# Youngju-Na/UFORecon

Hardware: AMD Instinct MI355X
Metric: rays/s (per-ray volume-rendering path, 64+64 hierarchical samples, DTU-shaped 3-view 512x640) (higher is better)
Workload: dtype f32; 1 GPU; configs[1]: full 512x640 frame = 327680 rays, 3 source views, 64+64 samples, rays sharded by row tiles over 1 GPU(s), depth/RGB tiles all-gathered; rays_per_frame=327680, chunk_rays=4096, side_streams=3

## Files before the change

### uforecon_amd/csrc/ray_transformer.hip

```cpp
#include "bwd_tape.h"
#include "ufr_internal.h"
#include "weight_stream_f16.h"

namespace ufr {

__device__ __forceinline__ void load_ray_tile(const float* __restrict__ token0, const int* __restrict__ tok_row,
                                              const float* __restrict__ order_pe, size_t tok_base, int s_base, int g,
                                              int j, f32x4 (&x)[6]) {
  const float* row = token0 + (tok_row ? (size_t)tok_row[tok_base + j] : tok_base + j) * UFR_TOKEN_DIM;
#pragma unroll
  for (int t = 0; t < 5; ++t) x[t] = ld4(row + 16 * t + 4 * g);
  const float* pe = order_pe + (size_t)(s_base + j) * 8 + 2 * g;
  x[5] = f32x4{pe[0], pe[1], 0.f, 0.f};
}

template <int VW, int VB, int C, class WS>
__device__ __forceinline__ void layer_norm88(f32x4 (&tt)[C][6], const WS& ws, int g, float eps, float asc, f32x4 (*XH)[6] = nullptr, float* RS = nullptr) {
#pragma unroll
  for (int c = 0; c < C; ++c) {
    f32x4 (&t)[6] = tt[c];
    float s = 0.f;
#pragma unroll
    for (int i = 0; i < 5; ++i) s += (t[i][0] + t[i][1]) + (t[i][2] + t[i][3]);
    s += t[5][0] + t[5][1];
    const float mean = sum_groups(s) * (1.f / 88.f);
    float q = 0.f;
#pragma unroll
    for (int i = 0; i < 6; ++i)
#pragma unroll
      for (int r = 0; r < 4; ++r) {
        if (i < 5 || r < 2) {
          float d = t[i][r] - mean;
          q = fmaf(d, d, q);
        }
      }
    const float rstd = fast_rsqrt(sum_groups(q) * (1.f / 88.f) + eps);
    if (RS) RS[c] = rstd * asc;
#pragma unroll
    for (int i = 0; i < 6; ++i) {
      const f32x4 gw = vec_frag<VW>(ws, i, g), gb = vec_frag<VB>(ws, i, g);
#pragma unroll
      for (int r = 0; r < 4; ++r) {
        const float xh = (t[i][r] - mean) * rstd;
        if (XH) XH[c][i][r] = (i == 5 && r >= 2) ? 0.f : xh;
        t[i][r] = xh * gw[r] + gb[r];
      }
    }
  }
}

constexpr int kRtBlock = 256;
constexpr int kRtMinW = 2;
constexpr int kRtWaves = kRtBlock / 64;

#ifdef UFR_PHASE_TIMING
__device__ unsigned long long g_rt_phase[32];
#define UFR_RT_PHASE(i)                                                                \
  {                                                                                    \
    const unsigned long long t_now = __builtin_readcyclecounter();                     \
    rt_acc[i] += t_now - rt_prev;                                                      \
    rt_prev = t_now;                                                                   \
  }
#else
#define UFR_RT_PHASE(i)
#endif

template <bool LOWP, bool TAPE = false>
__global__ void __launch_bounds__(kRtBlock, TAPE ? 2 : kRtMinW) ray_transformer_kernel(const float* __restrict__ packed,
                                                                  const float* __restrict__ token0,
                                                                  const int* __restrict__ tok_row,
                                                                  const float* __restrict__ order_pe, int RN, int SN,
                                                                  float* __restrict__ srdf,
                                                                  float* __restrict__ ray_out,
                                                                  int* __restrict__ status, float* __restrict__ tape = nullptr,
                                                                  float* __restrict__ ray_state = nullptr) {
  extern __shared__ __attribute__((aligned(16))) char smem[];
  auto ws = wstream_f16_begin<kRtWaves, LOWP>(packed, smem);
  wstream_f16_prime<B_RT1, kRtWaves>(ws);
  const int lane = threadIdx.x & 63, g = lane >> 4, j = lane & 15;
  const int ray_raw = (blockIdx.x * blockDim.x + threadIdx.x) >> 6;
  const bool valid = ray_raw < RN;
  const int ray = valid ? ray_raw : RN - 1;
  const int n_tiles = SN / 16;
  const int n_iter = n_tiles;
  const auto sc = scalar_file<false, ray_scalars_offset()>(ws);
  const float xs_x = sc[RS_XS_X];
  const float k_dsc = sc[RS_K_DSC], k_l2e = sc[RS_K_L2E], q_dsc = sc[RS_Q_DSC], q_l2e = sc[RS_Q_L2E];
  const float inv_len = uniform_f32(sc[RS_V_DSC] / (float)SN), f_len = uniform_f32((float)SN * sc[RS_V_ASC]);
  const bool pow2_len = (SN & (SN - 1)) == 0;

#ifdef UFR_PHASE_TIMING
  unsigned long long rt_acc[16] = {};
  unsigned long long rt_prev = __builtin_readcyclecounter();
#endif
  f32x4 KV[8], KVT[TAPE ? 8 : 1];
#pragma unroll
  for (int h = 0; h < 8; ++h) KV[h] = splat4(0.f);
#pragma unroll
  for (int h = 0; h < (TAPE ? 8 : 1); ++h) KVT[h] = splat4(0.f);
  for (int it = 0; it < n_iter; ++it) {
    constexpr int C = 1;
    const bool wrap = it + 1 < n_iter;
    const bool slot_ok = head11_slot(j) >= 0;
    f32x4 x[C][6], kt[C][8], vt[C][8];
    bool live[C];
#pragma unroll
    for (int c = 0; c < C; ++c) {
      const int tile = it * C + c;
      live[c] = tile < n_tiles;
      const int tl = live[c] ? tile : n_tiles - 1;
      load_ray_tile(token0, tok_row, order_pe, (size_t)ray * SN + tl * 16, tl * 16, g, j, x[c]);
#pragma unroll
      for (int h = 0; h < 8; ++h) { kt[c][h] = splat4(0.f); vt[c][h] = splat4(0.f); }
    }
    {
      BWords<C> cur;
      split_units<0, 0, 4 * C>(x, cur, xs_x);
      static_for<3>([&](auto si) __attribute__((always_inline)) {
        constexpr int s = decltype(si)::value;
        BStep b[C];
        bwords_to_bstep(cur, b);
        if constexpr (s < 2) {
          BWords<C> nxt;
          gemm_f16_panel<M_RT_K, s, C, kRtWaves, true>(ws, b, kt, wrap, [&](auto ti) __attribute__((always_inline)) {
            constexpr int to = decltype(ti)::value;
            split_units<s + 1, to * 4 * C / 8, (to + 1) * 4 * C / 8>(x, nxt, xs_x);
          });
          gemm_f16_panel<M_RT_V, s, C, kRtWaves, true>(ws, b, vt, wrap);
          cur = nxt;
        } else {
          gemm_f16_panel<M_RT_K, s, C, kRtWaves, true>(ws, b, kt, wrap);
          gemm_f16_panel<M_RT_V, s, C, kRtWaves, true>(ws, b, vt, wrap);
        }
      });
      probe_gemm(kt, ws);
      probe_gemm(vt, ws);
    }
    UFR_RT_PHASE(0)
    const float pad_v = (TAPE ? j == 3 : (j & 3) == 3) ? 1.f : 0.f;
#pragma unroll
    for (int c = 0; c < C; ++c) {
      float kk[8][4], vv[8][4];
      if (pow2_len) {
#pragma unroll
        for (int h = 0; h < 8; ++h)
#pragma unroll
          for (int r = 0; r < 4; ++r) vv[h][r] = vt[c][h][r] * inv_len;
      } else {
#pragma unroll
        for (int h = 0; h < 8; ++h)
#pragma unroll
          for (int r = 0; r < 4; ++r) vv[h][r] = vt[c][h][r] / f_len;
      }
      const bool k_ok = slot_ok && live[c];
#pragma unroll
      for (int h = 0; h < 8; ++h)
#pragma unroll
        for (int r = 0; r < 4; ++r) {
          const float e = elu1_acc(kt[c][h][r], k_dsc, k_l2e);
          kk[h][r] = k_ok ? e : 0.f;
          vv[h][r] = slot_ok ? vv[h][r] : pad_v;
        }
#pragma unroll
      for (int r = 0; r < 4; ++r) {
#pragma unroll
        for (int h = 0; h < 8; ++h) {
          KV[h] = mfma16(kk[h][r], vv[h][r], KV[h]);
          if constexpr (TAPE) KVT[h] = mfma16(vv[h][r], kk[h][r], KVT[h]);
        }
      }
    }
    wstream_f16_finish<B_RT1, kRtWaves>(ws, wrap);
    UFR_RT_PHASE(1)
  }

  if constexpr (TAPE) {
    if (valid) {
      float* st = ray_state + (size_t)ray * (kRayStateTiles * kTileFloats) + lane * 4;
#pragma unroll
      for (int h = 0; h < 8; ++h) { st4(st + h * kTileFloats, KV[h]); st4(st + (8 + h) * kTileFloats, KVT[h]); }
    }
  }
  wstream_f16_prime<B_RT2, kRtWaves>(ws);
  constexpr int C = 1;
  const int n_iter2 = TAPE ? n_iter + (n_iter & 1) : n_iter;
  typedef RayTapeLayout<LOWP> TapeL;
  for (int it = 0; it < n_iter2; ++it) {
    const bool wrap = it + 1 < n_iter2;
    char* const tape_blk = reinterpret_cast<char*>(tape) + ((size_t)ray * (n_iter2 / 2) + it / 2) * (TapeL::block_units * 512);
    auto tape_st = [&](int tile, f32x4 v) __attribute__((always_inline)) {
      if (valid) tile_store<TapeL>(tape_blk, tile, it & 1, lane, v);
    };
    f32x4 x[C][6], q[C][6], msg[C][6];
    bool live[C];
    int tbase[C];
#pragma unroll
    for (int c = 0; c < C; ++c) {
      const int tile = it * C + c;
      live[c] = tile < n_tiles;
      tbase[c] = (live[c] ? tile : n_tiles - 1) * 16;
      load_ray_tile(token0, tok_row, order_pe, (size_t)ray * SN + tbase[c], tbase[c], g, j, x[c]);
#pragma unroll
      for (int t = 0; t < 6; ++t) q[c][t] = splat4(0.f);
    }
    track_external(x, ws);
    gemm_f16<M_RT_Q, C, kRtWaves>(ws, x, q, wrap, xs_x);
    float zs_all[8];
    if constexpr (TAPE) {
#pragma unroll
      for (int t = 0; t < 6; ++t) {
        tape_st(RT_X + t, live[0] ? x[0][t] : splat4(0.f));
        f32x4 qq;
#pragma unroll
        for (int r = 0; r < 4; ++r) qq[r] = quad11(t, g, r) >= 0 ? elu1_acc(q[0][t][r], q_dsc, q_l2e) : 0.f;
        tape_st(RT_Q + t, qq);
      }
    }
    UFR_RT_PHASE(2)
#pragma unroll
    for (int c = 0; c < C; ++c) {
      static_for<8>([&](auto hi) __attribute__((always_inline)) {
        constexpr int h = decltype(hi)::value;
        f32x4 acc = splat4(0.f);
        static_for<3>([&](auto qi) __attribute__((always_inline)) {
          constexpr int qd = decltype(qi)::value, quad = 3 * h + qd;
          const float qq = (3 * g + qd < 11) ? elu1_acc(q[c][quad >> 2][quad & 3], q_dsc, q_l2e) : 0.f;
          acc = mfma16(KV[h][qd], qq, acc);
        });
        const float den = TAPE ? __shfl(acc[3], j) : acc[3];
        const float Z = fast_rcp(den + 1e-6f);
        const float zs = Z * (float)SN;
        if constexpr (TAPE) zs_all[h] = zs;
        static_for<3>([&](auto ri) __attribute__((always_inline)) {
          constexpr int rr = decltype(ri)::value, quad = 3 * h + rr;
          msg[c][quad >> 2][quad & 3] = acc[rr] * zs;
        });
      });
    }
    UFR_RT_PHASE(3)
    if constexpr (TAPE) {
#pragma unroll
      for (int t = 0; t < 6; ++t) tape_st(RT_MSG + t, msg[0][t]);
      tape_st(RT_ZS, f32x4{zs_all[0], zs_all[1], zs_all[2], zs_all[3]});
      tape_st(RT_ZS + 1, f32x4{zs_all[4], zs_all[5], zs_all[6], zs_all[7]});
    }
    f32x4 m[C][6];
#pragma unroll
    for (int c = 0; c < C; ++c)
#pragma unroll
      for (int t = 0; t < 6; ++t) m[c][t] = splat4(0.f);
    gemm_f16<M_RT_MERGE, C, kRtWaves>(ws, msg, m, wrap, sc[RS_M_XS]);
    UFR_RT_PHASE(4)
    float rstd1[C] = {}, rstd2[C] = {};
    if constexpr (TAPE) {
      f32x4 xh[C][6];
      layer_norm88<V_RT_N1W, V_RT_N1B, C>(m, ws, g, sc[RS_EPS1], sc[RS_M_ASC], xh, rstd1);
#pragma unroll
      for (int t = 0; t < 6; ++t) { tape_st(RT_XH1 + t, xh[0][t]); tape_st(RT_M + t, m[0][t]); }
    } else {
      layer_norm88<V_RT_N1W, V_RT_N1B, C>(m, ws, g, sc[RS_EPS1], 1.f);
    }
    UFR_RT_PHASE(5)

    f32x4 cat[C][12], hid[C][11], o[C][6];
#pragma unroll
    for (int c = 0; c < C; ++c) {
#pragma unroll
      for (int t = 0; t < 6; ++t) { cat[c][t] = x[c][t]; cat[c][6 + t] = m[c][t]; }
#pragma unroll
      for (int t = 0; t < 11; ++t) hid[c][t] = splat4(0.f);
    }
    gemm_f16<M_RT_MLP0, C, kRtWaves>(ws, cat, hid, wrap, xs_x);
    UFR_RT_PHASE(6)
#pragma unroll
    for (int c = 0; c < C; ++c) {
#pragma unroll
      for (int t = 0; t < 11; ++t)
#pragma unroll
        for (int r = 0; r < 4; ++r) hid[c][t][r] = relu_acc(hid[c][t][r]);
#pragma unroll
      for (int t = 0; t < 6; ++t) o[c][t] = splat4(0.f);
    }
    unsigned relu_bits[2] = {0u, 0u};
    if constexpr (TAPE) {
#pragma unroll
      for (int t = 0; t < 11; ++t) {
        tape_st(RT_HID + t, hid[0][t] * sc[RS_MLP0_DSC]);
#pragma unroll
        for (int r = 0; r < 4; ++r)
          if (hid[0][t][r] > 0.f) relu_bits[(4 * t + r) >> 5] |= 1u << ((4 * t + r) & 31);
      }
    }
    gemm_f16<M_RT_MLP2, C, kRtWaves>(ws, hid, o, wrap, sc[RS_M_MLP2]);
    UFR_RT_PHASE(7)
    if constexpr (TAPE) {
      f32x4 xh[C][6];
      layer_norm88<V_RT_N2W, V_RT_N2B, C>(o, ws, g, sc[RS_EPS2], sc[RS_MLP2_ASC], xh, rstd2);
#pragma unroll
      for (int t = 0; t < 6; ++t) tape_st(RT_XH2 + t, xh[0][t]);
    } else {
      layer_norm88<V_RT_N2W, V_RT_N2B, C>(o, ws, g, sc[RS_EPS2], 1.f);
    }
    UFR_RT_PHASE(8)
#pragma unroll
    for (int c = 0; c < C; ++c) {
#pragma unroll
      for (int t = 0; t < 6; ++t)
#pragma unroll
        for (int r = 0; r < 4; ++r) o[c][t][r] += x[c][t][r];
      if constexpr (TAPE) {
#pragma unroll
        for (int t = 0; t < 6; ++t) tape_st(RT_O + t, o[c][t]);
      }
      if (ray_out && valid && live[c]) {
        float* row = ray_out + ((size_t)ray * SN + tbase[c] + j) * UFR_RAY_DIM;
#pragma unroll
        for (int t = 0; t < 5; ++t) st4(row + 16 * t + 4 * g, o[c][t]);
        row[80 + 2 * g] = o[c][5][0];
        row[81 + 2 * g] = o[c][5][1];
      }
    }

    f32x4 d1[C][2], d2[C][1], d3[C][1];
#pragma unroll
    for (int c = 0; c < C; ++c) {
      d1[c][0] = vec_frag<V_DM_B0>(ws, 0, g) * sc[RS_DM0_ASC];
      d1[c][1] = vec_frag<V_DM_B0>(ws, 1, g) * sc[RS_DM0_ASC];
      d2[c][0] = vec_frag<V_DM_B2>(ws, 0, g) * sc[RS_DM2_ASC];
      d3[c][0] = vec_frag<V_DM_B4>(ws, 0, g) * sc[RS_DM4_ASC];
    }
    gemm_f16<M_DM0, C, kRtWaves>(ws, o, d1, wrap, sc[RS_DM0_XS]);
#pragma unroll
    for (int c = 0; c < C; ++c)
#pragma unroll
      for (int t = 0; t < 2; ++t)
#pragma unroll
        for (int r = 0; r < 4; ++r) d1[c][t][r] = relu_acc(d1[c][t][r]);
    gemm_f16<M_DM2, C, kRtWaves>(ws, d1, d2, wrap, sc[RS_M_DM2]);
#pragma unroll
    for (int c = 0; c < C; ++c)
#pragma unroll
      for (int r = 0; r < 4; ++r) d2[c][0][r] = relu_acc(d2[c][0][r]);
    if constexpr (TAPE) {
#pragma unroll
      for (int t = 0; t < 2; ++t) {
        tape_st(RT_D1 + t, d1[0][t] * sc[RS_DM0_DSC]);
#pragma unroll
        for (int r = 0; r < 4; ++r)
          if (d1[0][t][r] > 0.f) relu_bits[(44 + 4 * t + r) >> 5] |= 1u << ((44 + 4 * t + r) & 31);
      }
      tape_st(RT_D2, d2[0][0] * sc[RS_DM2_DSC]);
#pragma unroll
      for (int r = 0; r < 4; ++r)
        if (d2[0][0][r] > 0.f) relu_bits[1] |= 1u << (52 + r - 32);
      tape_st(RT_MISC, f32x4{rstd1[0], rstd2[0], __builtin_bit_cast(float, relu_bits[0]), __builtin_bit_cast(float, relu_bits[1])});
    }
    gemm_f16<M_DM4, C, kRtWaves>(ws, d2, d3, wrap, sc[RS_M_DM4]);
#pragma unroll
    for (int c = 0; c < C; ++c)
      if (g == 0 && valid && live[c]) srdf[(size_t)ray * SN + tbase[c] + j] = d3[c][0][0] * sc[RS_DM4_DSC];
    wstream_f16_finish<B_RT2, kRtWaves>(ws, wrap);
    UFR_RT_PHASE(9)
  }
  wstream_report_range(ws, status);
#ifdef UFR_PHASE_TIMING
  if (ray_raw == 5 && lane == 0)
    for (int i = 0; i < 16; ++i) g_rt_phase[i] += rt_acc[i];
#endif
}

template <bool LOWP, bool TAPE = false>
static hipError_t launch_rt(const float* packed, const float* token0, const int* tok_row, const float* order_pe, int RN,
                            int SN, float* srdf, float* ray_out, int* status, hipStream_t s, float* tape = nullptr,
                            float* ray_state = nullptr) {
  static LdsAttrOnce lds_attr;
  if (const hipError_t attr = lds_attr.set(reinterpret_cast<const void*>(&ray_transformer_kernel<LOWP, TAPE>), kF16LdsBytes); attr != hipSuccess) return attr;
  hipLaunchKernelGGL((ray_transformer_kernel<LOWP, TAPE>), dim3((RN + kRtWaves - 1) / kRtWaves), dim3(kRtBlock), kF16LdsBytes, s,
                     packed, token0, tok_row, order_pe, RN, SN, srdf, ray_out, status, tape, ray_state);
  return hipGetLastError();
}

hipError_t launch_ray_tape(const float* packed, const float* token0, const int* tok_row, const float* order_pe, int RN, int SN,
                           float* srdf, float* tape, float* ray_state, bool lowp, int* status, hipStream_t s) {
  if (SN % 16 != 0 || SN < 16) return hipErrorInvalidValue;
  return lowp ? launch_rt<true, true>(packed, token0, tok_row, order_pe, RN, SN, srdf, nullptr, status, s, tape, ray_state)
              : launch_rt<false, true>(packed, token0, tok_row, order_pe, RN, SN, srdf, nullptr, status, s, tape, ray_state);
}

hipError_t launch_ray_transformer(const float* packed, const float* token0, const int* tok_row, const float* order_pe,
                                  int RN, int SN, float* srdf, float* ray_out, bool lowp, int* status, hipStream_t s) {
  if (SN % 16 != 0 || SN < 16) return hipErrorInvalidValue;
  return lowp ? launch_rt<true>(packed, token0, tok_row, order_pe, RN, SN, srdf, ray_out, status, s)
              : launch_rt<false>(packed, token0, tok_row, order_pe, RN, SN, srdf, ray_out, status, s);
}

}

#ifdef UFR_PHASE_TIMING
extern "C" int ufr_debug_rt_phases(unsigned long long* out, int n, int reset) {
  unsigned long long h[32] = {};
  if (hipMemcpyFromSymbol(h, HIP_SYMBOL(ufr::g_rt_phase), sizeof(h)) != hipSuccess) return -1;
  for (int i = 0; i < n && i < 32; ++i) out[i] = h[i];
  if (reset) {
    unsigned long long z[32] = {};
    if (hipMemcpyToSymbol(HIP_SYMBOL(ufr::g_rt_phase), z, sizeof(z)) != hipSuccess) return -1;
  }
  return 0;
}
#endif
```

### uforecon_amd/csrc/ufr_layout_f16.h

```cpp
#pragma once
#include "ufr_layout.h"

namespace ufr {

constexpr int kPlanes = 2;
constexpr int kScaleExpWMin = -40, kScaleExpWMax = 24, kScaleExpXMin = -40, kScaleExpXMax = 12;
constexpr float kDefaultInputAbsMax = 4094.f;
constexpr int kF16ChunkFrags = 12;
constexpr int kF16Slots = 3;
constexpr int kF16Depth = 2;
static_assert(kF16Depth >= 1 && kF16Depth * kPlanes <= kF16ChunkFrags, "read-ahead must stay inside one chunk");

enum F16Stream { B_VT = 0, B_RT1 = 1, B_RT2 = 2, B_COUNT = 3, B_VTB = 3, B_RTB1 = 4, B_RTB2 = 5, B_ALL = 6 };
__host__ __device__ constexpr bool f16_mat_is_bf16(int m) { return m >= M_COUNT; }

struct Panel { int mat, s; };

__host__ __device__ constexpr int ksteps(int m) { return (mat_desc(m).n_in + 1) / 2; }

__host__ __device__ constexpr int f16_n_panels(int S) {
  return S == B_VT ? 3 * 3 + 3 + 5 + 5 + 3 + 1 + 1 : S == B_RT1 ? 6 : S == B_RT2 ? 3 + 3 + 6 + 6 + 3 + 1 + 1
       : S == B_VTB ? 1 + 1 + 3 + 5 + 3 + 3 * 3
       : S == B_RTB1 ? 1 + 1 + 3 + 6 + 3 + 3
       : 6 + 4 + 4;
}
__host__ __device__ constexpr Panel f16_panel(int S, int i) {
  if (S == B_VT) {
    if (i < 6) return {i % 2 == 0 ? M_VT_Q : M_VT_K, i / 2};
    if (i < 9) return {M_VT_V, i - 6};
    i -= 9;
    if (i < 3) return {M_VT_MERGE, i};
    i -= 3;
    if (i < 5) return {M_VT_MLP0, i};
    i -= 5;
    if (i < 5) return {M_VT_MLP2, i};
    i -= 5;
    if (i < 3) return {M_RW0, i};
    i -= 3;
    return {i == 0 ? M_RW2 : M_RW4, 0};
  }
  if (S == B_RT1) return {i % 2 == 0 ? M_RT_K : M_RT_V, i / 2};
  if (S == B_VTB) {
    if (i < 1) return {M_RW2T, 0};
    i -= 1;
    if (i < 1) return {M_RW0T, 0};
    i -= 1;
    if (i < 3) return {M_VT_MLP2T, i};
    i -= 3;
    if (i < 5) return {M_VT_MLP0T, i};
    i -= 5;
    if (i < 3) return {M_VT_MERGET, i};
    i -= 3;
    return {i < 3 ? M_VT_QT : i < 6 ? M_VT_KT : M_VT_VT, i % 3};
  }
  if (S == B_RTB1) {
    if (i < 1) return {M_DM2T, 0};
    i -= 1;
    if (i < 1) return {M_DM0T, 0};
    i -= 1;
    if (i < 3) return {M_RT_MLP2T, i};
    i -= 3;
    if (i < 6) return {M_RT_MLP0T, i};
    i -= 6;
    if (i < 3) return {M_RT_MERGET, i};
    i -= 3;
    return {M_RT_QT, i};
  }
  if (S == B_RTB2) {
    if (i < 6) return {i % 2 == 0 ? M_RT_K : M_RT_V, i / 2};
    i -= 6;
    return {i < 4 ? M_RT_KT : M_RT_VT, i % 4};
  }
  if (i < 3) return {M_RT_Q, i};
  i -= 3;
  if (i < 3) return {M_RT_MERGE, i};
  i -= 3;
  if (i < 6) return {M_RT_MLP0, i};
  i -= 6;
  if (i < 6) return {M_RT_MLP2, i};
  i -= 6;
  if (i < 3) return {M_DM0, i};
  i -= 3;
  return {i == 0 ? M_DM2 : M_DM4, 0};
}
__host__ __device__ constexpr int f16_mat_stream(int m) {
  return m >= M_DM2T ? ((m == M_RT_KT || m == M_RT_VT) ? B_RTB2 : B_RTB1)
         : m >= M_COUNT ? B_VTB
         : (m == M_RT_K || m == M_RT_V) ? B_RT1
         : (m == M_RT_Q || m == M_RT_MERGE || m == M_RT_MLP0 || m == M_RT_MLP2 || m == M_DM0 || m == M_DM2 || m == M_DM4)
             ? B_RT2
             : B_VT;
}
__host__ __device__ constexpr int f16_panel_frags(int S, int i) { return mat_desc(f16_panel(S, i).mat).n_out * kPlanes; }
__host__ __device__ constexpr int f16_panel_start(int S, int i) {
  int o = 0;
  for (int j = 0; j < i; ++j) o += f16_panel_frags(S, j);
  return o;
}
__host__ __device__ constexpr int f16_panel_index(int m, int s, int S = -1) {
  if (S < 0) S = f16_mat_stream(m);
  for (int i = 0; i < f16_n_panels(S); ++i)
    if (f16_panel(S, i).mat == m && f16_panel(S, i).s == s) return i;
  return -1;
}
__host__ __device__ constexpr int f16_stream_frags(int S) { return f16_panel_start(S, f16_n_panels(S)); }
__host__ __device__ constexpr int f16_stream_real_chunks(int S) { return (f16_stream_frags(S) + kF16ChunkFrags - 1) / kF16ChunkFrags; }
__host__ __device__ constexpr int f16_stream_chunks(int S) { return (f16_stream_real_chunks(S) + kF16Slots - 1) / kF16Slots * kF16Slots; }
__host__ __device__ constexpr int f16_stream_base_frags(int S) {
  int o = 0;
  for (int j = 0; j < S; ++j) o += f16_stream_chunks(j) * kF16ChunkFrags;
  return o;
}
constexpr int kF16FragsPadded = f16_stream_base_frags(B_COUNT);
constexpr int kF16Halfwords = kF16FragsPadded * 512;
constexpr int kF16Bytes = kF16FragsPadded * 1024;
constexpr int kBwdFragsPadded = f16_stream_base_frags(B_ALL) - kF16FragsPadded;
constexpr int kBwdHalfwords = kBwdFragsPadded * 512;
constexpr int kBwdBytes = kBwdFragsPadded * 1024;

__host__ __device__ constexpr int f16_col(int m, int s, int g, int i) {
  const MatDesc d = mat_desc(m);
  const int tile = 2 * s + (i >> 2);
  return tile < d.n_in ? col_map(d.cm, tile, g, i & 3, d.in_dim) : -1;
}

__host__ __device__ inline void plan_entry_f16(int h, int* param, int* elem, int* plane, int* is_bf16 = nullptr, int* mat = nullptr) {
  *param = -1; *elem = 0; *plane = 0;
  int f = h >> 9;
  const int lane = (h >> 3) & 63, i = h & 7;
  int S = 0;
  while (S + 1 < B_ALL && f >= f16_stream_base_frags(S + 1)) ++S;
  if (is_bf16) *is_bf16 = 0;
  if (mat) *mat = -1;
  f -= f16_stream_base_frags(S);
  if (f >= f16_stream_frags(S)) return;
  int pi = 0;
  while (f >= f16_panel_frags(S, pi)) { f -= f16_panel_frags(S, pi); ++pi; }
  const Panel p = f16_panel(S, pi);
  if (is_bf16) *is_bf16 = f16_mat_is_bf16(p.mat) ? 1 : 0;
  if (mat) *mat = p.mat;
  const MatDesc d = mat_desc(p.mat);
  const int to = f / kPlanes;
  *plane = f % kPlanes;
  const int row = row_map(d.rm, to, lane & 15, d.out_dim);
  const int col = f16_col(p.mat, p.s, lane >> 4, i);
  if (row >= 0 && col >= 0) { *param = d.param; *elem = d.trans ? col * d.k_raw + row : row * d.k_raw + col; }
}

}
```

### uforecon_amd/csrc/weight_stream_f16.h

```cpp
#pragma once
#include <type_traits>

#include "ufr_layout_f16.h"
#include "weight_stream.h"

namespace ufr {

typedef _Float16 f16x8 __attribute__((ext_vector_type(8)));
typedef _Float16 f16x2 __attribute__((ext_vector_type(2)));
typedef float f32x2 __attribute__((ext_vector_type(2)));
typedef unsigned u32x4 __attribute__((ext_vector_type(4)));
typedef int i32x4 __attribute__((ext_vector_type(4)));

constexpr int kF16RingBytes = kF16Slots * kF16ChunkFrags * 1024;
constexpr int kF16LdsBytes = kF16RingBytes + kVecBytes;

__device__ __forceinline__ void split_pair(float a, float b, float m, unsigned& h, unsigned& l) {
  if (__builtin_constant_p(a) && __builtin_constant_p(b) && a == 0.f && b == 0.f) {
    h = l = 0u;
    return;
  }
  asm("v_fma_mixlo_f16 %0, %1, %2, 0" : "=v"(h) : "v"(a), "s"(m));
  asm("v_fma_mixhi_f16 %0, %1, %2, 0" : "+v"(h) : "v"(b), "s"(m));
  asm("v_fma_mixlo_f16 %0, %1, %2, -%3 op_sel_hi:[0,0,1]" : "=v"(l) : "v"(a), "s"(m), "v"(h));
  asm("v_fma_mixhi_f16 %0, %1, %2, -%3 op_sel:[0,0,1] op_sel_hi:[0,0,1]" : "+v"(l) : "v"(b), "s"(m), "v"(h));
}

struct BStep { f16x8 p[kPlanes]; };

typedef __bf16 bf16x2 __attribute__((ext_vector_type(2)));
typedef __bf16 bf16x8 __attribute__((ext_vector_type(8)));
__device__ __forceinline__ void split_pair_bf16(float a, float b, unsigned& h, unsigned& l) {
  h = __builtin_bit_cast(unsigned, __builtin_convertvector(f32x2{a, b}, bf16x2));
  const float ah = __builtin_bit_cast(float, h << 16), bh = __builtin_bit_cast(float, h & 0xffff0000u);
  l = __builtin_bit_cast(unsigned, __builtin_convertvector(f32x2{a - ah, b - bh}, bf16x2));
}

template <bool LOWP, bool BF16 = false>
struct WStreamF16T {
  static constexpr bool lowp = LOWP;
  static constexpr bool bf16 = BF16;
  const char* src;
  char* ring;
  unsigned ring_lds;
  i32x4 rsrc;
  unsigned lds_wave;
  const f32x4* vecs;
  int wave, lane;
  unsigned long long bad_in, bad_out;
  f16x8 pre[kF16Depth][kPlanes];
};

typedef WStreamF16T<false> WStreamF16;
template <int NWAVES, bool LOWP = false, bool BF16 = false>
__device__ __forceinline__ WStreamF16T<LOWP, BF16> wstream_f16_begin(const float* __restrict__ packed, char* smem) {
  WStreamF16T<LOWP, BF16> ws;
  ws.lane = threadIdx.x & 63;
  ws.wave = __builtin_amdgcn_readfirstlane(threadIdx.x >> 6);
  ws.bad_in = ws.bad_out = 0ull;
  constexpr size_t kPlaneRegion = (size_t)blob_floats() * 4;
  ws.src = reinterpret_cast<const char*>(packed) + kPlaneRegion;
  ws.ring = smem;
  ws.ring_lds = __builtin_amdgcn_readfirstlane((unsigned)(size_t)(lds_ptr_t)smem);
  {
    const unsigned long long base = reinterpret_cast<unsigned long long>(ws.src) + (unsigned long long)ws.wave * 1024ull;
    ws.rsrc[0] = __builtin_amdgcn_readfirstlane((int)(unsigned)(base & 0xffffffffull));
    ws.rsrc[1] = __builtin_amdgcn_readfirstlane((int)(unsigned)((base >> 32) & 0xffffull));
    ws.rsrc[2] = -1;
    ws.rsrc[3] = 0x00020000;
    ws.lds_wave = ws.ring_lds + (unsigned)ws.wave * 1024u;
  }
  f32x4* v = reinterpret_cast<f32x4*>(smem + kF16RingBytes);
  ws.vecs = v;
  constexpr int voff = vec_region_offset(), n4 = vec_region_floats() / 4;
  const f32x4* vs = reinterpret_cast<const f32x4*>(packed + voff);
  for (int i = threadIdx.x; i < n4; i += NWAVES * 64) v[i] = vs[i];
  __syncthreads();
  return ws;
}

template <unsigned GOFF, unsigned LOFF>
__device__ __forceinline__ void lds_dma_piece(const i32x4& rsrc, unsigned lds_wave, unsigned lane_off) {
  unsigned soff;
  asm volatile("s_add_u32 m0, %3, %5\n\ts_mov_b32 %0, %4\n\tbuffer_load_dwordx4 %1, %2, %0 offen lds"
               : "=&s"(soff)
               : "v"(lane_off), "s"(rsrc), "s"(lds_wave), "n"(GOFF), "n"(LOFF)
               : "memory", "scc");
}

template <int S, int NWAVES, int CHK, int P0 = 0, int P1 = kF16ChunkFrags / NWAVES, class WS>
__device__ __forceinline__ void wstream_f16_fetch(const WS& ws) {
  static_assert(kF16ChunkFrags % NWAVES == 0, "chunk must split evenly over the fetching waves");
  if constexpr (P1 > P0) {
    constexpr size_t goff = ((size_t)f16_stream_base_frags(S) + (size_t)CHK * kF16ChunkFrags) * 1024;
    constexpr int soff = (CHK % kF16Slots) * (kF16ChunkFrags * 1024);
    const unsigned lane_off = ws.lane * 16;
    static_assert(goff + (size_t)kF16ChunkFrags * 1024 < (1ull << 31), "buffer offsets are 32-bit");
    static_for<P1 - P0>([&](auto ki) __attribute__((always_inline)) {
      constexpr unsigned k = P0 + decltype(ki)::value;
      lds_dma_piece<(unsigned)goff + k * NWAVES * 1024u, (unsigned)soff + k * NWAVES * 1024u>(ws.rsrc, ws.lds_wave, lane_off);
    });
  }
}

template <int S, int NWAVES, int CHK, class WS>
__device__ __forceinline__ void wstream_f16_barrier(const WS& ws, bool wrap) {
  constexpr int per_chunk = kF16ChunkFrags / NWAVES, ahead = kF16Slots - 1, n_chunks = f16_stream_chunks(S);
  constexpr int younger = (kF16Slots - 2) * per_chunk;
  if constexpr (younger == 0) {
    asm volatile("s_waitcnt vmcnt(0) lgkmcnt(0)" ::: "memory");
  } else if constexpr (CHK + ahead <= n_chunks) {
    asm volatile("s_waitcnt vmcnt(%0) lgkmcnt(0)" ::"n"(younger) : "memory");
  } else {
    if (wrap) asm volatile("s_waitcnt vmcnt(%0) lgkmcnt(0)" ::"n"(younger) : "memory");
    else asm volatile("s_waitcnt vmcnt(0) lgkmcnt(0)" ::: "memory");
  }
  __syncthreads();
}

template <int S, int NWAVES, int CHK, int P0 = 0, int P1 = kF16ChunkFrags / NWAVES, class WS>
__device__ __forceinline__ void wstream_f16_refill(const WS& ws, bool wrap) {
  constexpr int ahead = kF16Slots - 1, n_chunks = f16_stream_chunks(S);
  if constexpr (CHK + ahead < n_chunks) {
    wstream_f16_fetch<S, NWAVES, CHK + ahead, P0, P1>(ws);
  } else {
    if (wrap) wstream_f16_fetch<S, NWAVES, (CHK + ahead) % n_chunks, P0, P1>(ws);
  }
}

template <int S, int NWAVES, int CHK, class WS>
__device__ __forceinline__ void wstream_f16_open(const WS& ws, bool wrap) {
  wstream_f16_barrier<S, NWAVES, CHK>(ws, wrap);
  wstream_f16_refill<S, NWAVES, CHK>(ws, wrap);
}

template <int S, int NWAVES, class WS>
__device__ __forceinline__ void wstream_f16_finish(const WS& ws, bool wrap) {
  constexpr int real = f16_stream_real_chunks(S), pad = f16_stream_chunks(S) - real;
  static_for<pad>([&](auto ci) __attribute__((always_inline)) { wstream_f16_open<S, NWAVES, real + decltype(ci)::value>(ws, wrap); });
}

template <int S, int NWAVES, class WS>
__device__ __forceinline__ void wstream_f16_prime(const WS& ws) {
  static_for<kF16Slots - 1>([&](auto ci) __attribute__((always_inline)) { wstream_f16_fetch<S, NWAVES, decltype(ci)::value>(ws); });
}

template <int C, int N, class WS>
__device__ __forceinline__ void probe_gemm(const f32x4 (&out)[C][N], WS& ws) {
  bool bad = false;
#pragma unroll
  for (int c = 0; c < C; ++c) bad |= __builtin_amdgcn_class(out[c][0][0], 0x207);
  ws.bad_in |= __builtin_amdgcn_ballot_w64(bad);
}
template <int C, int N, class WS>
__device__ __forceinline__ void track_external(const f32x4 (&t)[C][N], WS& ws) {
  bool nan = false;
#pragma unroll
  for (int c = 0; c < C; ++c)
#pragma unroll
    for (int i = 0; i < N; ++i)
      nan |= __builtin_isunordered(t[c][i][0], t[c][i][1]) | __builtin_isunordered(t[c][i][2], t[c][i][3]);
  ws.bad_out |= __builtin_amdgcn_ballot_w64(nan);
}

template <class WS>
__device__ __forceinline__ void wstream_report_range(const WS& ws, int* __restrict__ status) {
  const int bits = (ws.bad_in ? 1 : 0) | (ws.bad_out ? 2 : 0);
  if (bits && ws.lane == 0) atomicOr(status, bits);
}

template <int V, class WS>
__device__ __forceinline__ f32x4 vec_frag(const WS& ws, int t, int g) {
  constexpr int base = (vec_offset(V) - vec_region_offset()) / 4;
  return ws.vecs[base + t * 4 + g];
}

__device__ __forceinline__ float uniform_f32(float v) {
  return __builtin_bit_cast(float, __builtin_amdgcn_readfirstlane(__builtin_bit_cast(int, v)));
}
template <bool LOCAL>
struct ScalarFile {
  float sv;
  __device__ __forceinline__ float operator[](int k) const {
    float v = sv;
    if constexpr (LOCAL) asm volatile("" : "+v"(v));
    return __builtin_bit_cast(float, __builtin_amdgcn_readlane(__builtin_bit_cast(int, v), k));
  }
};
template <bool LOCAL, int OFFSET, class WS>
__device__ __forceinline__ ScalarFile<LOCAL> scalar_file(const WS& ws) {
  constexpr int base = OFFSET - vec_region_offset();
  return ScalarFile<LOCAL>{reinterpret_cast<const float*>(ws.vecs)[base + (ws.lane & (kKernelScalars - 1))]};
}

__device__ __forceinline__ f32x4 mfma_f16(const f16x8& a, const f16x8& b, const f32x4& c) {
  return __builtin_amdgcn_mfma_f32_16x16x32_f16(a, b, c, 0, 0, 0);
}
template <bool BF>
__device__ __forceinline__ f32x4 mfma_planes(const f16x8& a, const f16x8& b, const f32x4& c) {
  if constexpr (BF)
    return __builtin_amdgcn_mfma_f32_16x16x32_bf16(__builtin_bit_cast(bf16x8, a), __builtin_bit_cast(bf16x8, b), c, 0, 0, 0);
  else
    return __builtin_amdgcn_mfma_f32_16x16x32_f16(a, b, c, 0, 0, 0);
}

constexpr int kHookValu = 6;
constexpr int kProducts = 3;
constexpr int kSetprio = 1;
struct NoHook {
  template <class T> __device__ __forceinline__ void operator()(T) const {}
};
template <int M, int S, int C, int NWAVES, bool SWAP = false, int STREAM = -1, class Hook = NoHook, class WS = WStreamF16>
__device__ __forceinline__ void gemm_f16_panel(WS& ws, const BStep (&b)[C], f32x4 (&out)[C][mat_desc(M).n_out],
                                              bool wrap, Hook&& hook = NoHook{}) {
  constexpr bool LOWP = WS::lowp;
  constexpr bool BF = f16_mat_is_bf16(M);
  constexpr int n_planes = LOWP ? 1 : kPlanes, n_products = LOWP ? 1 : kProducts;
  constexpr int n_out = mat_desc(M).n_out, ST = STREAM >= 0 ? STREAM : f16_mat_stream(M);
  static_assert(f16_panel_index(M, S, ST) >= 0, "not a panel of the stream");
  constexpr int F0 = f16_panel_start(ST, f16_panel_index(M, S, ST));
  const f16x8* lds = reinterpret_cast<const f16x8*>(ws.ring) + ws.lane;
  __builtin_amdgcn_s_setprio(kSetprio);
  static_for<n_out>([&](auto ti) __attribute__((always_inline)) {
    constexpr int to = decltype(ti)::value;
    constexpr int f = F0 + to * kPlanes;
    constexpr int sidx = f / kPlanes, n_stages = f16_stream_frags(ST) / kPlanes;
    __builtin_amdgcn_sched_barrier(0);
    auto read_stage = [&](auto si) __attribute__((always_inline)) {
      constexpr int s2 = decltype(si)::value, f2 = s2 * kPlanes;
      constexpr int chk = f2 / kF16ChunkFrags, in_chk = f2 % kF16ChunkFrags;
      constexpr int base = ((chk % kF16Slots) * kF16ChunkFrags + in_chk) * 64;
      constexpr int in_frags = f16_stream_frags(ST) - chk * kF16ChunkFrags;
      constexpr int n_st = (in_frags < kF16ChunkFrags ? in_frags : kF16ChunkFrags) / kPlanes, j = in_chk / kPlanes;
      constexpr int pieces = kF16ChunkFrags / NWAVES;
      if constexpr (in_chk == 0) wstream_f16_barrier<ST, NWAVES, chk>(ws, wrap);
      wstream_f16_refill<ST, NWAVES, chk, j * pieces / n_st, (j + 1) * pieces / n_st>(ws, wrap);
#pragma unroll
      for (int p = 0; p < n_planes; ++p) ws.pre[s2 % kF16Depth][p] = lds[base + p * 64];
    };
    if constexpr (sidx == 0)
      static_for<kF16Depth>([&](auto di) __attribute__((always_inline)) { read_stage(di); });
    f16x8 a[kPlanes];
#pragma unroll
    for (int p = 0; p < n_planes; ++p) a[p] = ws.pre[sidx % kF16Depth][p];
    if constexpr (sidx + kF16Depth < n_stages) read_stage(std::integral_constant<int, sidx + kF16Depth>{});
    __builtin_amdgcn_sched_barrier(0);
    hook(ti);
#pragma unroll
    for (int c = 0; c < C; ++c)
      static_for<n_products>([&](auto pi) __attribute__((always_inline)) {
        constexpr int pw[kProducts] = {1, 0, 0}, px[kProducts] = {0, 1, 0};
        constexpr int w = LOWP ? 0 : pw[decltype(pi)::value], x = LOWP ? 0 : px[decltype(pi)::value];
        out[c][to] = SWAP ? mfma_planes<BF>(b[c].p[x], a[w], out[c][to]) : mfma_planes<BF>(a[w], b[c].p[x], out[c][to]);
      });
    if constexpr (!std::is_same<std::decay_t<Hook>, NoHook>::value) {
#pragma unroll
      for (int i = 0; i < n_products * C; ++i) {
        __builtin_amdgcn_sched_group_barrier(0x008, 1, 0);
        __builtin_amdgcn_sched_group_barrier(0x002, kHookValu, 0);
      }
    }
#pragma unroll
    for (int c = 0; c < C; ++c) asm volatile("" : "+v"(out[c][to]));
  });
  __builtin_amdgcn_sched_barrier(0);
  __builtin_amdgcn_s_setprio(0);
}

template <int C>
struct BWords { unsigned w[C][kPlanes][4]; };

template <int S, int U0, int U1, bool BF = false, int C, int NIN>
__device__ __forceinline__ void split_units(const f32x4 (&in)[C][NIN], BWords<C>& bw, float m) {
  static_for<U1 - U0>([&](auto ui) __attribute__((always_inline)) {
    constexpr int u = U0 + decltype(ui)::value;
    constexpr int c = u / 4, half = (u >> 1) & 1, q = u & 1, tile = 2 * S + half;
    if constexpr (tile < NIN) {
      if constexpr (BF) split_pair_bf16(in[c][tile][2 * q], in[c][tile][2 * q + 1], bw.w[c][0][2 * half + q], bw.w[c][1][2 * half + q]);
      else split_pair(in[c][tile][2 * q], in[c][tile][2 * q + 1], m, bw.w[c][0][2 * half + q], bw.w[c][1][2 * half + q]);
    } else {
      bw.w[c][0][2 * half + q] = bw.w[c][1][2 * half + q] = 0u;
    }
  });
}

template <int C>
__device__ __forceinline__ void bwords_to_bstep(const BWords<C>& bw, BStep (&b)[C]) {
#pragma unroll
  for (int c = 0; c < C; ++c)
#pragma unroll
    for (int p = 0; p < kPlanes; ++p)
      b[c].p[p] = __builtin_bit_cast(f16x8, u32x4{bw.w[c][p][0], bw.w[c][p][1], bw.w[c][p][2], bw.w[c][p][3]});
}

__device__ __forceinline__ float elu1_acc(float a, float dsc, float dsc_l2e) {
  return a > 0.f ? __builtin_fmaf(a, dsc, 1.f) : __builtin_amdgcn_exp2f(dsc_l2e * a);
}
constexpr float kLog2e = 0x1.715476p+0f;

template <int M, int C, int NWAVES, int STREAM = -1, int NIN, class WS, class UHook = NoHook>
__device__ __forceinline__ void gemm_f16(WS& ws, const f32x4 (&in)[C][NIN], f32x4 (&out)[C][mat_desc(M).n_out],
                                        bool wrap, float m = 1.f, UHook&& uhook = NoHook{}) {
  static_assert(NIN == mat_desc(M).n_in, "input tile count");
  constexpr int n_out = mat_desc(M).n_out, NU = 4 * C;
  constexpr bool BF = f16_mat_is_bf16(M);
  constexpr bool kUser = !std::is_same<std::decay_t<UHook>, NoHook>::value;
  BWords<C> cur;
  split_units<0, 0, NU, BF>(in, cur, m);
  static_for<ksteps(M)>([&](auto si) __attribute__((always_inline)) {
    constexpr int s = decltype(si)::value;
    BStep b[C];
    bwords_to_bstep(cur, b);
    if constexpr (s + 1 < ksteps(M) && n_out >= 2) {
      BWords<C> nxt;
      gemm_f16_panel<M, s, C, NWAVES, false, STREAM>(ws, b, out, wrap, [&](auto ti) __attribute__((always_inline)) {
        constexpr int to = decltype(ti)::value;
        split_units<s + 1, to * NU / n_out, (to + 1) * NU / n_out, BF>(in, nxt, m);
        if constexpr (kUser) uhook(std::integral_constant<int, s * n_out + to>{});
      });
      cur = nxt;
    } else if constexpr (kUser) {
      gemm_f16_panel<M, s, C, NWAVES, false, STREAM>(ws, b, out, wrap, [&](auto ti) __attribute__((always_inline)) {
        uhook(std::integral_constant<int, s * n_out + decltype(ti)::value>{});
      });
      if constexpr (s + 1 < ksteps(M)) split_units<s + 1, 0, NU, BF>(in, cur, m);
    } else {
      gemm_f16_panel<M, s, C, NWAVES, false, STREAM>(ws, b, out, wrap);
      if constexpr (s + 1 < ksteps(M)) split_units<s + 1, 0, NU, BF>(in, cur, m);
    }
  });
  if constexpr (!BF) probe_gemm(out, ws);
}

}
```

Before: 2.604 million rays/s.

## Process two ray tiles per weight pass in RT1 with head-grouped virtual weight order

In the non-tape ray transformer first stage, each weight-stream pass now handles two 16-sample tiles (C=2) instead of one, and loops over head groups of two. The B_RT1 weight stream is fetched in a permuted virtual order so each head group's K/V panels arrive contiguously. This is meant to halve weight-streaming traffic and barrier count per tile while keeping accumulator register pressure bounded. The stream barriers also now skip padding pieces and compute exact vmcnt waits. The risks are added register pressure from C=2 and added complexity in the fetch and wait accounting.

```diff
diff --git a/uforecon_amd/csrc/ray_transformer.hip b/uforecon_amd/csrc/ray_transformer.hip
--- a/uforecon_amd/csrc/ray_transformer.hip
+++ b/uforecon_amd/csrc/ray_transformer.hip
@@ -75,7 +75,7 @@
                                                                   int* __restrict__ status, float* __restrict__ tape = nullptr,
                                                                   float* __restrict__ ray_state = nullptr) {
   extern __shared__ __attribute__((aligned(16))) char smem[];
-  auto ws = wstream_f16_begin<kRtWaves, LOWP>(packed, smem);
+  auto ws = wstream_f16_begin<kRtWaves, LOWP, false, !TAPE>(packed, smem);
   wstream_f16_prime<B_RT1, kRtWaves>(ws);
   const int lane = threadIdx.x & 63, g = lane >> 4, j = lane & 15;
   const int ray_raw = (blockIdx.x * blockDim.x + threadIdx.x) >> 6;
@@ -98,80 +98,150 @@
   for (int h = 0; h < 8; ++h) KV[h] = splat4(0.f);
 #pragma unroll
   for (int h = 0; h < (TAPE ? 8 : 1); ++h) KVT[h] = splat4(0.f);
-  for (int it = 0; it < n_iter; ++it) {
-    constexpr int C = 1;
-    const bool wrap = it + 1 < n_iter;
+  if constexpr (TAPE) {
+    for (int it = 0; it < n_iter; ++it) {
+      constexpr int C = 1;
+      const bool wrap = it + 1 < n_iter;
+      const bool slot_ok = head11_slot(j) >= 0;
+      f32x4 x[C][6], kt[C][8], vt[C][8];
+      bool live[C];
+#pragma unroll
+      for (int c = 0; c < C; ++c) {
+        const int tile = it * C + c;
+        live[c] = tile < n_tiles;
+        const int tl = live[c] ? tile : n_tiles - 1;
+        load_ray_tile(token0, tok_row, order_pe, (size_t)ray * SN + tl * 16, tl * 16, g, j, x[c]);
+#pragma unroll
+        for (int h = 0; h < 8; ++h) { kt[c][h] = splat4(0.f); vt[c][h] = splat4(0.f); }
+      }
+      {
+        BWords<C> cur;
+        split_units<0, 0, 4 * C>(x, cur, xs_x);
+        static_for<3>([&](auto si) __attribute__((always_inline)) {
+          constexpr int s = decltype(si)::value;
+          BStep b[C];
+          bwords_to_bstep(cur, b);
+          if constexpr (s < 2) {
+            BWords<C> nxt;
+            gemm_f16_panel<M_RT_K, s, C, kRtWaves, true>(ws, b, kt, wrap, [&](auto ti) __attribute__((always_inline)) {
+              constexpr int to = decltype(ti)::value;
+              split_units<s + 1, to * 4 * C / 8, (to + 1) * 4 * C / 8>(x, nxt, xs_x);
+            });
+            gemm_f16_panel<M_RT_V, s, C, kRtWaves, true>(ws, b, vt, wrap);
+            cur = nxt;
+          } else {
+            gemm_f16_panel<M_RT_K, s, C, kRtWaves, true>(ws, b, kt, wrap);
+            gemm_f16_panel<M_RT_V, s, C, kRtWaves, true>(ws, b, vt, wrap);
+          }
+        });
+        probe_gemm(kt, ws);
+        probe_gemm(vt, ws);
+      }
+      UFR_RT_PHASE(0)
+      const float pad_v = (TAPE ? j == 3 : (j & 3) == 3) ? 1.f : 0.f;
+#pragma unroll
+      for (int c = 0; c < C; ++c) {
+        float kk[8][4], vv[8][4];
+        if (pow2_len) {
+#pragma unroll
+          for (int h = 0; h < 8; ++h)
+#pragma unroll
+            for (int r = 0; r < 4; ++r) vv[h][r] = vt[c][h][r] * inv_len;
+        } else {
+#pragma unroll
+          for (int h = 0; h < 8; ++h)
+#pragma unroll
+            for (int r = 0; r < 4; ++r) vv[h][r] = vt[c][h][r] / f_len;
+        }
+        const bool k_ok = slot_ok && live[c];
+#pragma unroll
+        for (int h = 0; h < 8; ++h)
+#pragma unroll
+          for (int r = 0; r < 4; ++r) {
+            const float e = elu1_acc(kt[c][h][r], k_dsc, k_l2e);
+            kk[h][r] = k_ok ? e : 0.f;
+            vv[h][r] = slot_ok ? vv[h][r] : pad_v;
+          }
+#pragma unroll
+        for (int r = 0; r < 4; ++r) {
+#pragma unroll
+          for (int h = 0; h < 8; ++h) {
+            KV[h] = mfma16(kk[h][r], vv[h][r], KV[h]);
+            if constexpr (TAPE) KVT[h] = mfma16(vv[h][r], kk[h][r], KVT[h]);
+          }
+        }
+      }
+      wstream_f16_finish<B_RT1, kRtWaves>(ws, wrap);
+      UFR_RT_PHASE(1)
+    }
+  } else {
     const bool slot_ok = head11_slot(j) >= 0;
-    f32x4 x[C][6], kt[C][8], vt[C][8];
-    bool live[C];
-#pragma unroll
-    for (int c = 0; c < C; ++c) {
-      const int tile = it * C + c;
-      live[c] = tile < n_tiles;
-      const int tl = live[c] ? tile : n_tiles - 1;
-      load_ray_tile(token0, tok_row, order_pe, (size_t)ray * SN + tl * 16, tl * 16, g, j, x[c]);
-#pragma unroll
-      for (int h = 0; h < 8; ++h) { kt[c][h] = splat4(0.f); vt[c][h] = splat4(0.f); }
-    }
-    {
-      BWords<C> cur;
-      split_units<0, 0, 4 * C>(x, cur, xs_x);
-      static_for<3>([&](auto si) __attribute__((always_inline)) {
-        constexpr int s = decltype(si)::value;
-        BStep b[C];
-        bwords_to_bstep(cur, b);
-        if constexpr (s < 2) {
-          BWords<C> nxt;
-          gemm_f16_panel<M_RT_K, s, C, kRtWaves, true>(ws, b, kt, wrap, [&](auto ti) __attribute__((always_inline)) {
-            constexpr int to = decltype(ti)::value;
-            split_units<s + 1, to * 4 * C / 8, (to + 1) * 4 * C / 8>(x, nxt, xs_x);
-          });
-          gemm_f16_panel<M_RT_V, s, C, kRtWaves, true>(ws, b, vt, wrap);
-          cur = nxt;
-        } else {
-          gemm_f16_panel<M_RT_K, s, C, kRtWaves, true>(ws, b, kt, wrap);
-          gemm_f16_panel<M_RT_V, s, C, kRtWaves, true>(ws, b, vt, wrap);
+    const float pad_v = (j & 3) == 3 ? 1.f : 0.f;
+    auto pass = [&](auto cc, int tile0, bool wrap) __attribute__((always_inline)) {
+      constexpr int C = decltype(cc)::value, G = kRt1GroupHeads;
+      BWords<C> bw[3];
+      {
+        f32x4 x[C][6];
+#pragma unroll
+        for (int c = 0; c < C; ++c)
+          load_ray_tile(token0, tok_row, order_pe, (size_t)ray * SN + (tile0 + c) * 16, (tile0 + c) * 16, g, j, x[c]);
+        static_for<3>([&](auto si) __attribute__((always_inline)) {
+          constexpr int s = decltype(si)::value;
+          split_units<s, 0, 4 * C>(x, bw[s], xs_x);
+        });
+      }
+      static_for<kRt1Heads / G>([&](auto gi) __attribute__((always_inline)) {
+        constexpr int H0 = decltype(gi)::value * G;
+        f32x4 kt[C][G], vt[C][G];
+#pragma unroll
+        for (int c = 0; c < C; ++c)
+#pragma unroll
+          for (int h = 0; h < G; ++h) { kt[c][h] = splat4(0.f); vt[c][h] = splat4(0.f); }
+        static_for<3>([&](auto si) __attribute__((always_inline)) {
+          constexpr int s = decltype(si)::value;
+          BStep b[C];
+          bwords_to_bstep(bw[s], b);
+          gemm_f16_panel<M_RT_K, s, C, kRtWaves, true, -1, H0, G>(ws, b, kt, wrap);
+          gemm_f16_panel<M_RT_V, s, C, kRtWaves, true, -1, H0, G>(ws, b, vt, wrap);
+        });
+        if constexpr (H0 == 0) {
+          probe_gemm(kt, ws);
+          probe_gemm(vt, ws);
         }
+        UFR_RT_PHASE(0)
+#pragma unroll
+        for (int c = 0; c < C; ++c) {
+          float kk[G][4], vv[G][4];
+          if (pow2_len) {
+#pragma unroll
+            for (int h = 0; h < G; ++h)
+#pragma unroll
+              for (int r = 0; r < 4; ++r) vv[h][r] = vt[c][h][r] * inv_len;
+          } else {
+#pragma unroll
+            for (int h = 0; h < G; ++h)
+#pragma unroll
+              for (int r = 0; r < 4; ++r) vv[h][r] = vt[c][h][r] / f_len;
+          }
+#pragma unroll
+          for (int h = 0; h < G; ++h)
+#pragma unroll
+            for (int r = 0; r < 4; ++r) {
+              const float e = elu1_acc(kt[c][h][r], k_dsc, k_l2e);
+              kk[h][r] = slot_ok ? e : 0.f;
+              vv[h][r] = slot_ok ? vv[h][r] : pad_v;
+            }
+#pragma unroll
+          for (int r = 0; r < 4; ++r)
+#pragma unroll
+            for (int h = 0; h < G; ++h) KV[H0 + h] = mfma16(kk[h][r], vv[h][r], KV[H0 + h]);
+        }
+        UFR_RT_PHASE(1)
       });
-      probe_gemm(kt, ws);
-      probe_gemm(vt, ws);
-    }
-    UFR_RT_PHASE(0)
-    const float pad_v = (TAPE ? j == 3 : (j & 3) == 3) ? 1.f : 0.f;
-#pragma unroll
-    for (int c = 0; c < C; ++c) {
-      float kk[8][4], vv[8][4];
-      if (pow2_len) {
-#pragma unroll
-        for (int h = 0; h < 8; ++h)
-#pragma unroll
-          for (int r = 0; r < 4; ++r) vv[h][r] = vt[c][h][r] * inv_len;
-      } else {
-#pragma unroll
-        for (int h = 0; h < 8; ++h)
-#pragma unroll
-          for (int r = 0; r < 4; ++r) vv[h][r] = vt[c][h][r] / f_len;
-      }
-      const bool k_ok = slot_ok && live[c];
-#pragma unroll
-      for (int h = 0; h < 8; ++h)
-#pragma unroll
-        for (int r = 0; r < 4; ++r) {
-          const float e = elu1_acc(kt[c][h][r], k_dsc, k_l2e);
-          kk[h][r] = k_ok ? e : 0.f;
-          vv[h][r] = slot_ok ? vv[h][r] : pad_v;
-        }
-#pragma unroll
-      for (int r = 0; r < 4; ++r) {
-#pragma unroll
-        for (int h = 0; h < 8; ++h) {
-          KV[h] = mfma16(kk[h][r], vv[h][r], KV[h]);
-          if constexpr (TAPE) KVT[h] = mfma16(vv[h][r], kk[h][r], KVT[h]);
-        }
-      }
-    }
-    wstream_f16_finish<B_RT1, kRtWaves>(ws, wrap);
-    UFR_RT_PHASE(1)
+      wstream_f16_finish<B_RT1, kRtWaves>(ws, wrap);
+    };
+    for (int it = 0; it < n_tiles / 2; ++it) pass(std::integral_constant<int, 2>{}, 2 * it, 2 * it + 2 < n_tiles);
+    if (n_tiles & 1) pass(std::integral_constant<int, 1>{}, n_tiles - 1, false);
   }
 
   if constexpr (TAPE) {
diff --git a/uforecon_amd/csrc/ufr_layout_f16.h b/uforecon_amd/csrc/ufr_layout_f16.h
--- a/uforecon_amd/csrc/ufr_layout_f16.h
+++ b/uforecon_amd/csrc/ufr_layout_f16.h
@@ -111,6 +111,44 @@
   for (int j = 0; j < S; ++j) o += f16_stream_chunks(j) * kF16ChunkFrags;
   return o;
 }
+__host__ __device__ constexpr bool f16_stream_skips_padding(int S) { return S < B_COUNT; }
+
+constexpr int kRt1GroupHeads = 2;
+constexpr int kRt1Heads = 8;
+constexpr int kRt1GroupFrags = 6 * kRt1GroupHeads * kPlanes;
+__host__ __device__ constexpr int f16_rt1_virtual_to_blob(int v) {
+  const int run = kRt1GroupHeads * kPlanes;
+  const int gr = v / kRt1GroupFrags, r = v % kRt1GroupFrags, panel = r / run, q = r % run;
+  return panel * (kRt1Heads * kPlanes) + gr * run + q;
+}
+__host__ __device__ constexpr int f16_rt1_virtual_start(int pi, int to) {
+  return (to / kRt1GroupHeads) * kRt1GroupFrags + pi * (kRt1GroupHeads * kPlanes) + (to % kRt1GroupHeads) * kPlanes;
+}
+__host__ __device__ constexpr bool f16_rt1_map_ok() {
+  if (kRt1Heads % kRt1GroupHeads != 0 || (kRt1GroupHeads * kPlanes) % 4 != 0) return false;
+  if (mat_desc(M_RT_K).n_out != kRt1Heads || mat_desc(M_RT_V).n_out != kRt1Heads) return false;
+  if (f16_stream_frags(B_RT1) != 6 * kRt1Heads * kPlanes) return false;
+  bool seen[6 * kRt1Heads * kPlanes] = {};
+  for (int v = 0; v < f16_stream_frags(B_RT1); ++v) {
+    const int b = f16_rt1_virtual_to_blob(v);
+    if (b < 0 || b >= f16_stream_frags(B_RT1) || seen[b]) return false;
+    seen[b] = true;
+    if (v % 4 != 0 && b != f16_rt1_virtual_to_blob(v - 1) + 1) return false;
+  }
+  for (int pi = 0; pi < 6; ++pi)
+    for (int to = 0; to < kRt1Heads; ++to)
+      for (int p = 0; p < kPlanes; ++p)
+        if (f16_rt1_virtual_to_blob(f16_rt1_virtual_start(pi, to) + p) != f16_panel_start(B_RT1, pi) + to * kPlanes + p) return false;
+  return true;
+}
+static_assert(f16_rt1_map_ok(), "B_RT1's virtual order must permute the stream and keep every 4-fragment piece group contiguous");
+__host__ __device__ constexpr int f16_fetch_frag(int S, int v, bool vorder) {
+  return (vorder && S == B_RT1) ? f16_rt1_virtual_to_blob(v) : v;
+}
+__host__ __device__ constexpr int f16_stage_frag(int S, int pi, int to, bool vorder) {
+  return (vorder && S == B_RT1) ? f16_rt1_virtual_start(pi, to) : f16_panel_start(S, pi) + to * kPlanes;
+}
+
 constexpr int kF16FragsPadded = f16_stream_base_frags(B_COUNT);
 constexpr int kF16Halfwords = kF16FragsPadded * 512;
 constexpr int kF16Bytes = kF16FragsPadded * 1024;
diff --git a/uforecon_amd/csrc/weight_stream_f16.h b/uforecon_amd/csrc/weight_stream_f16.h
--- a/uforecon_amd/csrc/weight_stream_f16.h
+++ b/uforecon_amd/csrc/weight_stream_f16.h
@@ -36,10 +36,11 @@
   l = __builtin_bit_cast(unsigned, __builtin_convertvector(f32x2{a - ah, b - bh}, bf16x2));
 }
 
-template <bool LOWP, bool BF16 = false>
+template <bool LOWP, bool BF16 = false, bool VORDER = false>
 struct WStreamF16T {
   static constexpr bool lowp = LOWP;
   static constexpr bool bf16 = BF16;
+  static constexpr bool vorder = VORDER;
   const char* src;
   char* ring;
   unsigned ring_lds;
@@ -52,9 +53,9 @@
 };
 
 typedef WStreamF16T<false> WStreamF16;
-template <int NWAVES, bool LOWP = false, bool BF16 = false>
-__device__ __forceinline__ WStreamF16T<LOWP, BF16> wstream_f16_begin(const float* __restrict__ packed, char* smem) {
-  WStreamF16T<LOWP, BF16> ws;
+template <int NWAVES, bool LOWP = false, bool BF16 = false, bool VORDER = false>
+__device__ __forceinline__ WStreamF16T<LOWP, BF16, VORDER> wstream_f16_begin(const float* __restrict__ packed, char* smem) {
+  WStreamF16T<LOWP, BF16, VORDER> ws;
   ws.lane = threadIdx.x & 63;
   ws.wave = __builtin_amdgcn_readfirstlane(threadIdx.x >> 6);
   ws.bad_in = ws.bad_out = 0ull;
@@ -88,32 +89,58 @@
                : "memory", "scc");
 }
 
+template <int S, int NWAVES>
+__host__ __device__ constexpr bool f16_piece_issued(int chk, int k) {
+  return !f16_stream_skips_padding(S) || chk * kF16ChunkFrags + k * NWAVES < f16_stream_frags(S);
+}
+template <int S, int NWAVES>
+__host__ __device__ constexpr int f16_chunk_pieces(int chk) {
+  int n = 0;
+  for (int k = 0; k < kF16ChunkFrags / NWAVES; ++k) n += f16_piece_issued<S, NWAVES>(chk, k) ? 1 : 0;
+  return n;
+}
+
 template <int S, int NWAVES, int CHK, int P0 = 0, int P1 = kF16ChunkFrags / NWAVES, class WS>
 __device__ __forceinline__ void wstream_f16_fetch(const WS& ws) {
   static_assert(kF16ChunkFrags % NWAVES == 0, "chunk must split evenly over the fetching waves");
+  static_assert(!f16_stream_skips_padding(S) || f16_stream_frags(S) % NWAVES == 0, "a piece must be all weights or all padding");
   if constexpr (P1 > P0) {
-    constexpr size_t goff = ((size_t)f16_stream_base_frags(S) + (size_t)CHK * kF16ChunkFrags) * 1024;
+    constexpr size_t gbase = (size_t)f16_stream_base_frags(S) * 1024;
     constexpr int soff = (CHK % kF16Slots) * (kF16ChunkFrags * 1024);
     const unsigned lane_off = ws.lane * 16;
-    static_assert(goff + (size_t)kF16ChunkFrags * 1024 < (1ull << 31), "buffer offsets are 32-bit");
+    static_assert(gbase + (size_t)f16_stream_chunks(S) * kF16ChunkFrags * 1024 < (1ull << 31), "buffer offsets are 32-bit");
     static_for<P1 - P0>([&](auto ki) __attribute__((always_inline)) {
       constexpr unsigned k = P0 + decltype(ki)::value;
-      lds_dma_piece<(unsigned)goff + k * NWAVES * 1024u, (unsigned)soff + k * NWAVES * 1024u>(ws.rsrc, ws.lds_wave, lane_off);
+      if constexpr (f16_piece_issued<S, NWAVES>(CHK, k)) {
+        constexpr int v0 = CHK * kF16ChunkFrags + k * NWAVES;
+        constexpr int b0 = f16_fetch_frag(S, v0, WS::vorder);
+        static_assert(f16_fetch_frag(S, v0 + NWAVES - 1, WS::vorder) == b0 + NWAVES - 1, "a piece group must be contiguous in the blob");
+        lds_dma_piece<(unsigned)(gbase + (size_t)b0 * 1024), (unsigned)soff + k * NWAVES * 1024u>(ws.rsrc, ws.lds_wave, lane_off);
+      }
     });
   }
 }
 
 template <int S, int NWAVES, int CHK, class WS>
 __device__ __forceinline__ void wstream_f16_barrier(const WS& ws, bool wrap) {
-  constexpr int per_chunk = kF16ChunkFrags / NWAVES, ahead = kF16Slots - 1, n_chunks = f16_stream_chunks(S);
-  constexpr int younger = (kF16Slots - 2) * per_chunk;
-  if constexpr (younger == 0) {
-    asm volatile("s_waitcnt vmcnt(0) lgkmcnt(0)" ::: "memory");
-  } else if constexpr (CHK + ahead <= n_chunks) {
-    asm volatile("s_waitcnt vmcnt(%0) lgkmcnt(0)" ::"n"(younger) : "memory");
+  constexpr int n_chunks = f16_stream_chunks(S);
+  constexpr int younger_pass = [] {
+    int n = 0;
+    for (int i = 1; i <= kF16Slots - 2; ++i)
+      if (CHK + i < n_chunks) n += f16_chunk_pieces<S, NWAVES>(CHK + i);
+    return n;
+  }();
+  constexpr int younger_wrap = [] {
+    int n = 0;
+    for (int i = 1; i <= kF16Slots - 2; ++i)
+      if (CHK + i >= n_chunks) n += f16_chunk_pieces<S, NWAVES>((CHK + i) % n_chunks);
+    return n;
+  }();
+  if constexpr (younger_wrap == 0) {
+    asm volatile("s_waitcnt vmcnt(%0) lgkmcnt(0)" ::"n"(younger_pass) : "memory");
   } else {
-    if (wrap) asm volatile("s_waitcnt vmcnt(%0) lgkmcnt(0)" ::"n"(younger) : "memory");
-    else asm volatile("s_waitcnt vmcnt(0) lgkmcnt(0)" ::: "memory");
+    if (wrap) asm volatile("s_waitcnt vmcnt(%0) lgkmcnt(0)" ::"n"(younger_pass + younger_wrap) : "memory");
+    else asm volatile("s_waitcnt vmcnt(%0) lgkmcnt(0)" ::"n"(younger_pass) : "memory");
   }
   __syncthreads();
 }
@@ -210,20 +237,21 @@
 struct NoHook {
   template <class T> __device__ __forceinline__ void operator()(T) const {}
 };
-template <int M, int S, int C, int NWAVES, bool SWAP = false, int STREAM = -1, class Hook = NoHook, class WS = WStreamF16>
-__device__ __forceinline__ void gemm_f16_panel(WS& ws, const BStep (&b)[C], f32x4 (&out)[C][mat_desc(M).n_out],
+template <int M, int S, int C, int NWAVES, bool SWAP = false, int STREAM = -1, int T0 = 0, int NT = mat_desc(M).n_out, class Hook = NoHook, class WS = WStreamF16>
+__device__ __forceinline__ void gemm_f16_panel(WS& ws, const BStep (&b)[C], f32x4 (&out)[C][NT],
                                               bool wrap, Hook&& hook = NoHook{}) {
   constexpr bool LOWP = WS::lowp;
   constexpr bool BF = f16_mat_is_bf16(M);
   constexpr int n_planes = LOWP ? 1 : kPlanes, n_products = LOWP ? 1 : kProducts;
-  constexpr int n_out = mat_desc(M).n_out, ST = STREAM >= 0 ? STREAM : f16_mat_stream(M);
+  constexpr int ST = STREAM >= 0 ? STREAM : f16_mat_stream(M);
   static_assert(f16_panel_index(M, S, ST) >= 0, "not a panel of the stream");
-  constexpr int F0 = f16_panel_start(ST, f16_panel_index(M, S, ST));
+  static_assert(T0 >= 0 && NT >= 1 && T0 + NT <= mat_desc(M).n_out, "out tile range");
+  constexpr int PI = f16_panel_index(M, S, ST);
   const f16x8* lds = reinterpret_cast<const f16x8*>(ws.ring) + ws.lane;
   __builtin_amdgcn_s_setprio(kSetprio);
-  static_for<n_out>([&](auto ti) __attribute__((always_inline)) {
+  static_for<NT>([&](auto ti) __attribute__((always_inline)) {
     constexpr int to = decltype(ti)::value;
-    constexpr int f = F0 + to * kPlanes;
+    constexpr int f = f16_stage_frag(ST, PI, T0 + to, WS::vorder);
     constexpr int sidx = f / kPlanes, n_stages = f16_stream_frags(ST) / kPlanes;
     __builtin_amdgcn_sched_barrier(0);
     auto read_stage = [&](auto si) __attribute__((always_inline)) {
```

Result: faster. 2.640 million rays/s, median of 6 (+1.4%).
